# acbull/pyHGT

Hardware: AMD Instinct MI355X
Metric: HGTConv forward edges/sec (higher is better)
Workload: dtype f32 (typed linears and relation transforms as 3-term fp16 hi/lo MFMA with power-of-two row scales, fp32 accumulate)

## Files before the change

pyhgt_amd/csrc/hgt_edge_logits.hip:

```cpp
#include "hgt_edge_common.h"

#ifndef HGT_LOGITS_XCD
#define HGT_LOGITS_XCD 1
#endif

namespace {

template <int VEC, int LPH, bool RTE, bool S32 = false>
__global__ __launch_bounds__(256) void k_edge_logits(
    const HgtItem* __restrict__ items, const HgtPlanHeader* __restrict__ hdr, const int32_t* __restrict__ esrc,
    const int32_t* __restrict__ edst, const uint16_t* __restrict__ ertei, const float* __restrict__ Q,
    const float* __restrict__ K, const float* __restrict__ rteK, const float* __restrict__ attT, float* __restrict__ logits, int R,
    int HT, int rel_lo, int rel_hi, int item_lo, int item_hi, int items_cap) {
    constexpr int DKP = VEC * LPH, DP = 64 * VEC, H = 64 / LPH, UN = RTE ? (unroll_for<VEC>() * 3) / 4 : unroll_for<VEC>();
    const int hg = S32 ? 0 : blockIdx.y;
    if constexpr (S32) HT = H;
    const int64_t ld = S32 ? (int64_t)DP : (int64_t)HT * DKP;
    const int co = hg * DP;
    constexpr bool HOIST = (DKP * VEC <= 128);
    __shared__ __attribute__((aligned(16))) float s_bounce[4][DP + 4 * (64 / LPH)];

    const int lane = threadIdx.x & 63;
    const int wib = __builtin_amdgcn_readfirstlane(threadIdx.x >> 6);
#if HGT_LOGITS_XCD
    constexpr int XC = 16;
    const int q8 = (int)(blockIdx.x >> 3), vblock = (q8 / XC) * (8 * XC) + (int)(blockIdx.x & 7u) * XC + (q8 % XC);
#else
    const int vblock = blockIdx.x;
#endif
    const int item = item_lo + vblock * 4 + wib;
    const HgtItem it = items[min(item, items_cap - 1)];
    const int n_items = item_hi >= 0 ? item_hi : hdr->n_items;
    if (item >= n_items) return;
    const int beg = __builtin_amdgcn_readfirstlane(it.beg), end = __builtin_amdgcn_readfirstlane(it.end);
    const int rel = __builtin_amdgcn_readfirstlane(it.rel);
    const int h = lane / LPH, p = lane % LPH;
    if (rel < rel_lo || rel >= rel_hi) return;

    if (rel >= R) {
        for (int64_t i = (int64_t)beg * H + lane; i < (int64_t)end * H; i += 64) logits[(i / H) * HT + hg * H + (i % H)] = 0.0f;
        return;
    }

    float* bounce = s_bounce[wib];
    const float* __restrict__ fglob = attT + ((int64_t)(rel * HT + hg * H + h) * DKP) * DKP + p * VEC;
    float frag[HOIST ? DKP : 1][VEC];
    if constexpr (HOIST) {
#pragma unroll
        for (int j = 0; j < DKP; ++j) load_vec<VEC>(fglob + j * DKP, frag[j]);
    }

    int cur_dst = -1;
    float qt[VEC];
#pragma unroll
    for (int i = 0; i < VEC; ++i) qt[i] = 0.0f;

    constexpr int HB = UN / 2;
    for (int base = beg; base < end; base += 64) {
        const int nb = min(64, end - base);
        const int li = base + min(lane, nb - 1);
        const int my_src = esrc[li], my_dst = edst[li];
        const int my_rte = RTE ? (int)ertei[li] : 0;
        float krA[HB][VEC], qrA[HB][VEC], trA[RTE ? HB : 1][VEC];
        float krB[HB][VEC], qrB[HB][VEC], trB[RTE ? HB : 1][VEC];
#define HGT_ISSUE(KR, QR, TR, I0)                                                                  \
    _Pragma("unroll") for (int u = 0; u < HB; ++u) {                                               \
        const int idx = min((I0) + u, nb - 1);                                                     \
        const int s_ = __builtin_amdgcn_readlane(my_src, idx);                                     \
        const int d_ = __builtin_amdgcn_readlane(my_dst, idx);                                     \
        if constexpr (S32) {                                                                       \
            load_vec<VEC>(reinterpret_cast<const float*>(reinterpret_cast<const char*>(K) + (unsigned)((unsigned)s_ * (unsigned)(DP * 4) + (unsigned)(lane * VEC * 4))), KR[u]); \
            if constexpr (RTE) {                                                                   \
                const int ri = __builtin_amdgcn_readlane(my_rte, idx);                             \
                load_vec<VEC>(reinterpret_cast<const float*>(reinterpret_cast<const char*>(rteK) + (unsigned)((unsigned)ri * (unsigned)(DP * 4) + (unsigned)(lane * VEC * 4))), TR[u]); \
            }                                                                                      \
            load_vec<VEC>(reinterpret_cast<const float*>(reinterpret_cast<const char*>(Q) + (unsigned)((unsigned)d_ * (unsigned)(DP * 4) + (unsigned)(lane * VEC * 4))), QR[u]); \
        } else {                                                                                   \
            load_vec<VEC>(K + (int64_t)s_ * ld + co + lane * VEC, KR[u]);                          \
            if constexpr (RTE) {                                                                   \
                const int ri = __builtin_amdgcn_readlane(my_rte, idx);                             \
                load_vec<VEC>(rteK + (int64_t)ri * ld + co + lane * VEC, TR[u]);                   \
            }                                                                                      \
            load_vec<VEC>(Q + (int64_t)d_ * ld + co + lane * VEC, QR[u]);                          \
        }                                                                                          \
    }
#define HGT_PROCESS(KR, QR, TR, I0)                                                                \
    _Pragma("unroll") for (int u = 0; u < HB; ++u) {                                               \
        if ((I0) + u < nb) {                                                                       \
            const int d_ = __builtin_amdgcn_readlane(my_dst, (I0) + u);                            \
            if (d_ != cur_dst) {                                                                   \
                head_matvec<VEC, DKP, HOIST>(QR[u], bounce, lane, h, frag, fglob, qt);             \
                cur_dst = d_;                                                                      \
            }                                                                                      \
            float part = 0.0f;                                                                     \
            _Pragma("unroll") for (int i = 0; i < VEC; ++i) {                                      \
                float kv = KR[u][i];                                                               \
                if constexpr (RTE) kv += TR[u][i];                                                 \
                part = fmaf(qt[i], kv, part);                                                      \
            }                                                                                      \
            part = head_allreduce<LPH>(part);                                                      \
            if (p == 0) logits[(int64_t)(base + (I0) + u) * HT + hg * H + h] = part;               \
        }                                                                                          \
    }
        cur_dst = -1;
        HGT_ISSUE(krA, qrA, trA, 0)
        for (int i0 = 0; i0 < nb; i0 += 2 * HB) {
            HGT_ISSUE(krB, qrB, trB, i0 + HB)
            HGT_PROCESS(krA, qrA, trA, i0)
            HGT_ISSUE(krA, qrA, trA, i0 + 2 * HB)
            HGT_PROCESS(krB, qrB, trB, i0 + HB)
        }
#undef HGT_ISSUE
#undef HGT_PROCESS
    }
}

__global__ __launch_bounds__(256) void k_edge_softmax(const int32_t* __restrict__ segptr, float* __restrict__ s, int64_t NQ,
                                                      int H, int R) {
    const int64_t idx = (int64_t)blockIdx.x * blockDim.x + threadIdx.x;
    const int64_t dst = idx / H;
    const int h = (int)(idx % H);
    if (dst >= NQ) return;
    const int64_t tile = dst / HGT_TD, dl = dst % HGT_TD;
    float m = -INFINITY;
    for (int r = 0; r <= R; ++r) {
        const int64_t b = (tile * (R + 1) + r) * HGT_TD + dl;
        const int e0 = segptr[b], e1 = segptr[b + 1];
        for (int e = e0; e < e1; ++e) m = fmaxf(m, s[(int64_t)e * H + h]);
    }
    float z = 0.0f;
    for (int r = 0; r <= R; ++r) {
        const int64_t b = (tile * (R + 1) + r) * HGT_TD + dl;
        const int e0 = segptr[b], e1 = segptr[b + 1];
        for (int e = e0; e < e1; ++e) z += expf(s[(int64_t)e * H + h] - m);
    }
    const float inv = 1.0f / (z + 1e-16f);
    for (int r = 0; r <= R; ++r) {
        const int64_t b = (tile * (R + 1) + r) * HGT_TD + dl;
        const int e0 = segptr[b], e1 = segptr[b + 1];
        for (int e = e0; e < e1; ++e) {
            const int64_t o = (int64_t)e * H + h;
            s[o] = expf(s[o] - m) * inv;
        }
    }
}

__global__ void k_att_export(const int32_t* __restrict__ eid, const float* __restrict__ att, float* __restrict__ out, int64_t E, int H,
                             int Hout) {
    const int64_t i = (int64_t)blockIdx.x * blockDim.x + threadIdx.x;
    if (i >= E * H) return;
    const int64_t p = i / H;
    const int h = (int)(i % H);
    if (h < Hout) out[(int64_t)eid[p] * Hout + h] = att[i];
}

__global__ void k_relation_pack(const float* __restrict__ ratt, const float* __restrict__ rmsg, const float* __restrict__ rpri,
                                int R, int H, int HL, int dk, int dkp, float* __restrict__ attT, float* __restrict__ msgP) {
    const int64_t i = (int64_t)blockIdx.x * blockDim.x + threadIdx.x;
    const int64_t total = (int64_t)R * HL * dkp * dkp;
    if (i >= total) return;
    const int b = (int)(i % dkp), a = (int)((i / dkp) % dkp);
    const int64_t rhl = i / ((int64_t)dkp * dkp);
    const int hh = (int)(rhl % HL);
    const int64_t rh = (rhl / HL) * H + hh;
    float va = 0.0f, vm = 0.0f;
    if (a < dk && b < dk && hh < H) {
        va = ratt[(rh * dk + b) * dk + a] * rpri[rh] / sqrtf((float)dk);
        vm = rmsg[(rh * dk + a) * dk + b];
    }
    attT[i] = va;
    msgP[i] = vm;
}

template <int VEC, int LPH>
struct LaunchLogits {
    static int run(const HgtPlanView& pv, const float* Q, const float* K, const float* rteK, const float* attT, float* logits,
                   int R, int HT, int rel_lo, int rel_hi, int item_lo, int item_hi, int small32, hipStream_t stream) {
        const int64_t n_launch = item_hi >= 0 ? (int64_t)(item_hi - item_lo) : pv.L.max_items;
        const unsigned blocks = ((unsigned)((n_launch + 3) / 4) + 127u) & ~127u;
        dim3 grid(blocks, (unsigned)(HT / (64 / LPH)));
        if (small32 && grid.y == 1) {
            if (rteK)
                k_edge_logits<VEC, LPH, true, true><<<grid, 256, 0, stream>>>(pv.items, pv.hdr, pv.esrc, pv.edst, pv.ertei, Q, K, rteK, attT, logits, R, HT, rel_lo, rel_hi, item_lo, item_hi, (int)pv.L.max_items);
            else
                k_edge_logits<VEC, LPH, false, true><<<grid, 256, 0, stream>>>(pv.items, pv.hdr, pv.esrc, pv.edst, pv.ertei, Q, K, rteK, attT, logits, R, HT, rel_lo, rel_hi, item_lo, item_hi, (int)pv.L.max_items);
        } else if (rteK)
            k_edge_logits<VEC, LPH, true><<<grid, 256, 0, stream>>>(pv.items, pv.hdr, pv.esrc, pv.edst, pv.ertei, Q, K, rteK, attT, logits, R, HT, rel_lo, rel_hi, item_lo, item_hi, (int)pv.L.max_items);
        else
            k_edge_logits<VEC, LPH, false><<<grid, 256, 0, stream>>>(pv.items, pv.hdr, pv.esrc, pv.edst, pv.ertei, Q, K, rteK, attT, logits, R, HT, rel_lo, rel_hi, item_lo, item_hi, (int)pv.L.max_items);
        return HGT_OK;
    }
};

}

extern "C" int hgt_relation_pack(const float* relation_att, const float* relation_msg, const float* relation_pri,
                                 int32_t R, int32_t H, int32_t HL, int32_t d_k, int32_t dk_pad, float* att_t, float* msg_p, void* stream) {
    if (!relation_att || !relation_msg || !relation_pri || !att_t || !msg_p || R <= 0 || H <= 0 || HL < H || d_k <= 0 || dk_pad < d_k)
        return HGT_ERR_INVALID_ARG;
    const int64_t total = (int64_t)R * HL * dk_pad * dk_pad;
    k_relation_pack<<<(unsigned)((total + 255) / 256), 256, 0, (hipStream_t)stream>>>(relation_att, relation_msg, relation_pri, R, H, HL,
                                                                                      d_k, dk_pad, att_t, msg_p);
    HGT_CHECK_LAUNCH();
    return HGT_OK;
}

int hgt_launch_logits_mfma(int vec, int lph, int mode, const HgtPlanView& pv, const float* Q, const float* K, const float* rteK,
                           const unsigned short* attF, float* logits, int R, int HT, int rel_lo, int rel_hi, int item_lo, int item_hi, hipStream_t stream);

static int mfma_logits_split_for(int vec_full, int lph_full) {
    int s = 1;
    while (vec_full / s > 4 && lph_full * s * 2 <= 64) s *= 2;
    return (vec_full / s <= 4) ? s : 0;
}

static int edge_logits_impl(const void* plan, int64_t N, int64_t E, int32_t T, int32_t R, int32_t H, int32_t dk_pad, const float* Q,
                            const float* K, const float* rte_k, const float* att_t, float* logits, int rel_lo, int rel_hi, void* stream,
                            const void* att_frag = nullptr, int frag_f16 = 0, int item_lo = 0, int item_hi = -1) {
    if (!plan || !Q || !K || !att_t || !logits || H <= 0 || 64 % H != 0 || dk_pad <= 0) return HGT_ERR_INVALID_ARG;
    if (rel_lo < 0 || rel_hi > R + 1 || rel_lo > rel_hi) return HGT_ERR_INVALID_ARG;
    if (E == 0) return HGT_OK;
    const int lph = 64 / H;
    if (dk_pad % lph != 0) return HGT_ERR_INVALID_ARG;
    HgtPlanView pv = hgt_plan_view(plan, N, E, T, R);
    if (att_frag) {
        const int spm = mfma_logits_split_for(dk_pad / lph, lph);
        if (spm != 0) {
            int rc = hgt_launch_logits_mfma(dk_pad / lph / spm, lph * spm, (frag_f16 & 7) | (hgt_item_edges(E) << 8), pv, Q, K, rte_k, (const unsigned short*)att_frag,
                                            logits, (int)R, (int)H, rel_lo, rel_hi, item_lo, item_hi, (hipStream_t)stream);
            if (rc == HGT_OK) HGT_CHECK_LAUNCH();
            if (rc != HGT_ERR_UNSUPPORTED) return rc;
        }
    }
    const int sp = head_split_for(dk_pad / lph, lph, dk_pad);
    const int small32 = ((uint64_t)N * (uint64_t)H * (uint64_t)dk_pad * 4u < (1ull << 32)) ? 1 : 0;
    int rc = dispatch_layout<LaunchLogits>(dk_pad / lph / sp, lph * sp, pv, Q, K, rte_k, att_t, logits, (int)R, (int)H, rel_lo, rel_hi,
                                           item_lo, item_hi, small32, (hipStream_t)stream);
    if (rc != HGT_OK) return rc;
    HGT_CHECK_LAUNCH();
    return HGT_OK;
}

extern "C" int hgt_edge_logits(const void* plan, int64_t N, int64_t E, int32_t T, int32_t R, int32_t H, int32_t dk_pad,
                               const float* Q, const float* K, const float* rte_k, const float* att_t, float* logits, void* stream) {
    return edge_logits_impl(plan, N, E, T, R, H, dk_pad, Q, K, rte_k, att_t, logits, 0, R + 1, stream);
}

extern "C" int hgt_edge_logits_mfma(const void* plan, int64_t N, int64_t E, int32_t T, int32_t R, int32_t H, int32_t dk_pad,
                                    const float* Q, const float* K, const float* rte_k, const float* att_t, const void* att_frag,
                                    int32_t frag_f16, float* logits, void* stream) {
    if (!att_frag) return HGT_ERR_INVALID_ARG;
    return edge_logits_impl(plan, N, E, T, R, H, dk_pad, Q, K, rte_k, att_t, logits, 0, R + 1, stream, att_frag, frag_f16);
}

extern "C" int hgt_edge_logits_slice(const void* plan, int64_t N, int64_t E, int32_t T, int32_t R, int32_t H, int32_t dk_pad,
                                     const float* Q, const float* K, const float* rte_k, const float* att_t, float* logits,
                                     int32_t rel_lo, int32_t rel_hi, void* stream) {
    return edge_logits_impl(plan, N, E, T, R, H, dk_pad, Q, K, rte_k, att_t, logits, rel_lo, rel_hi, stream);
}

extern "C" int hgt_edge_logits_range(const void* plan, int64_t N, int64_t E, int32_t T, int32_t R, int32_t H, int32_t dk_pad,
                                     const float* Q, const float* K, const float* rte_k, const float* att_t, const void* att_frag,
                                     int32_t frag_f16, float* logits, int32_t item_begin, int32_t item_end, void* stream) {
    if (item_begin < 0 || item_end < item_begin) return HGT_ERR_INVALID_ARG;
    if (item_begin == item_end) return HGT_OK;
    return edge_logits_impl(plan, N, E, T, R, H, dk_pad, Q, K, rte_k, att_t, logits, 0, R + 1, stream, att_frag, frag_f16, item_begin, item_end);
}

extern "C" int hgt_edge_softmax(const void* plan, int64_t N, int64_t E, int32_t T, int32_t R, int32_t H, float* logits_att,
                                void* stream) {
    if (!plan || !logits_att || H <= 0) return HGT_ERR_INVALID_ARG;
    if (E == 0 || N == 0) return HGT_OK;
    HgtPlanView pv = hgt_plan_view(plan, N, E, T, R);
    const int64_t threads = N * H;
    k_edge_softmax<<<(unsigned)((threads + 255) / 256), 256, 0, (hipStream_t)stream>>>(pv.segptr, logits_att, N, H, R);
    HGT_CHECK_LAUNCH();
    return HGT_OK;
}


extern "C" int hgt_att_export(const void* plan, int64_t N, int64_t E, int32_t T, int32_t R, int32_t H, const float* att_sorted,
                              float* att_out, int32_t H_out, void* stream) {
    if (!plan || !att_sorted || !att_out || H <= 0 || H_out <= 0 || H_out > H) return HGT_ERR_INVALID_ARG;
    if (E == 0) return HGT_OK;
    HgtPlanView pv = hgt_plan_view(plan, N, E, T, R);
    k_att_export<<<(unsigned)((E * H + 255) / 256), 256, 0, (hipStream_t)stream>>>(pv.eid, att_sorted, att_out, E, H, H_out);
    HGT_CHECK_LAUNCH();
    return HGT_OK;
}
```

Measured before the change: 1.447 billion.

## Precompute dst-segment starts via DPP ballot and batch logit stores across lanes

Dst-change detection now happens once per 64-edge chunk: a DPP shift compares each lane's destination with the previous lane's, and a ballot gives a mask of segment starts. This replaces the per-edge readlane and compare in the inner loop. The full-chunk loop no longer clamps or bounds-checks indices, and a separate tail block handles a partial chunk. Logit stores are collected in a per-lane register across LPH consecutive edges and written as one store by all lanes of a head, instead of one p==0 lane-masked store per edge. This cuts scalar work and store instructions, but adds code size and a more complex tail path.

```diff
diff --git a/pyhgt_amd/csrc/hgt_edge_logits.hip b/pyhgt_amd/csrc/hgt_edge_logits.hip
--- a/pyhgt_amd/csrc/hgt_edge_logits.hip
+++ b/pyhgt_amd/csrc/hgt_edge_logits.hip
@@ -50,22 +50,25 @@
         for (int j = 0; j < DKP; ++j) load_vec<VEC>(fglob + j * DKP, frag[j]);
     }
 
-    int cur_dst = -1;
     float qt[VEC];
 #pragma unroll
     for (int i = 0; i < VEC; ++i) qt[i] = 0.0f;
 
     constexpr int HB = UN / 2;
+    const unsigned st_off = (unsigned)((p * HT + hg * H + h) * 4);
     for (int base = beg; base < end; base += 64) {
         const int nb = min(64, end - base);
         const int li = base + min(lane, nb - 1);
         const int my_src = esrc[li], my_dst = edst[li];
         const int my_rte = RTE ? (int)ertei[li] : 0;
+        const int prev_dst = __builtin_amdgcn_update_dpp(-1, my_dst, 0x138, 0xF, 0xF, false);
+        const uint64_t starts = __ballot(my_dst != prev_dst) | 1ull;
+        float sel = 0.0f;
         float krA[HB][VEC], qrA[HB][VEC], trA[RTE ? HB : 1][VEC];
         float krB[HB][VEC], qrB[HB][VEC], trB[RTE ? HB : 1][VEC];
-#define HGT_ISSUE(KR, QR, TR, I0)                                                                  \
+#define HGT_ISSUE(KR, QR, TR, I0, CLAMP)                                                           \
     _Pragma("unroll") for (int u = 0; u < HB; ++u) {                                               \
-        const int idx = min((I0) + u, nb - 1);                                                     \
+        const int idx = (CLAMP) ? min((I0) + u, nb - 1) : (I0) + u;                                \
         const int s_ = __builtin_amdgcn_readlane(my_src, idx);                                     \
         const int d_ = __builtin_amdgcn_readlane(my_dst, idx);                                     \
         if constexpr (S32) {                                                                       \
@@ -84,34 +87,45 @@
             load_vec<VEC>(Q + (int64_t)d_ * ld + co + lane * VEC, QR[u]);                          \
         }                                                                                          \
     }
-#define HGT_PROCESS(KR, QR, TR, I0)                                                                \
-    _Pragma("unroll") for (int u = 0; u < HB; ++u) {                                               \
-        if ((I0) + u < nb) {                                                                       \
-            const int d_ = __builtin_amdgcn_readlane(my_dst, (I0) + u);                            \
-            if (d_ != cur_dst) {                                                                   \
-                head_matvec<VEC, DKP, HOIST>(QR[u], bounce, lane, h, frag, fglob, qt);             \
-                cur_dst = d_;                                                                      \
+#define HGT_STORE_GROUP(J0) *reinterpret_cast<float*>(reinterpret_cast<char*>(logits + (int64_t)(base + (J0)) * HT) + st_off) = sel;
+#define HGT_PROCESS(KR, QR, TR, I0, TAIL)                                                          \
+    {                                                                                              \
+        const unsigned sm = (unsigned)(starts >> (I0));                                            \
+        _Pragma("unroll") for (int u = 0; u < HB; ++u) {                                           \
+            const int j = (I0) + u, jm = j & (LPH - 1);                                            \
+            if (!(TAIL) || j < nb) {                                                               \
+                if ((sm >> u) & 1u) head_matvec<VEC, DKP, HOIST>(QR[u], bounce, lane, h, frag, fglob, qt); \
+                float part = 0.0f;                                                                 \
+                _Pragma("unroll") for (int i = 0; i < VEC; ++i) {                                  \
+                    float kv = KR[u][i];                                                           \
+                    if constexpr (RTE) kv += TR[u][i];                                             \
+                    part = fmaf(qt[i], kv, part);                                                  \
+                }                                                                                  \
+                part = head_allreduce<LPH>(part);                                                  \
+                sel = (p == jm) ? part : sel;                                                      \
+                if (jm == LPH - 1) HGT_STORE_GROUP(j - jm)                                         \
             }                                                                                      \
-            float part = 0.0f;                                                                     \
-            _Pragma("unroll") for (int i = 0; i < VEC; ++i) {                                      \
-                float kv = KR[u][i];                                                               \
-                if constexpr (RTE) kv += TR[u][i];                                                 \
-                part = fmaf(qt[i], kv, part);                                                      \
-            }                                                                                      \
-            part = head_allreduce<LPH>(part);                                                      \
-            if (p == 0) logits[(int64_t)(base + (I0) + u) * HT + hg * H + h] = part;               \
         }                                                                                          \
     }
-        cur_dst = -1;
-        HGT_ISSUE(krA, qrA, trA, 0)
-        for (int i0 = 0; i0 < nb; i0 += 2 * HB) {
-            HGT_ISSUE(krB, qrB, trB, i0 + HB)
-            HGT_PROCESS(krA, qrA, trA, i0)
-            HGT_ISSUE(krA, qrA, trA, i0 + 2 * HB)
-            HGT_PROCESS(krB, qrB, trB, i0 + HB)
+        HGT_ISSUE(krA, qrA, trA, 0, false)
+        const int n_full = nb / (2 * HB);
+        for (int blk = 0; blk < n_full; ++blk) {
+            const int i0 = blk * (2 * HB);
+            HGT_ISSUE(krB, qrB, trB, i0 + HB, false)
+            HGT_PROCESS(krA, qrA, trA, i0, false)
+            HGT_ISSUE(krA, qrA, trA, (i0 + 2 * HB) & 63, false)
+            HGT_PROCESS(krB, qrB, trB, i0 + HB, false)
         }
+        if (n_full * (2 * HB) < nb) {
+            const int i0 = n_full * (2 * HB);
+            HGT_ISSUE(krB, qrB, trB, i0 + HB, true)
+            HGT_PROCESS(krA, qrA, trA, i0, true)
+            HGT_PROCESS(krB, qrB, trB, i0 + HB, true)
+        }
+        if ((nb & (LPH - 1)) != 0 && p < (nb & (LPH - 1))) HGT_STORE_GROUP(nb & ~(LPH - 1))
 #undef HGT_ISSUE
 #undef HGT_PROCESS
+#undef HGT_STORE_GROUP
     }
 }
 
```

Result: no change. 1.454 billion (median of 6 runs) (+0.5%).
